# 9vvqaq/Indoor-Point-Cloud-Datasets-Controllable-Generation-Method-for-Mobile-Robots-3D-Scene-Perception

Measured on AMD Instinct MI355X. Metric: rays/sec (whole node), 32-line x 2048-azimuth sweep, higher is better.
Workload: dtype f32

## Files before the change

### indoor-point-cloud-datasets-controllable-generation-method-for-mobile-robots-3d-scene-perception_amd/csrc/lidarcast.hip

```cpp
#include <hip/hip_runtime.h>

#include <chrono>
#include <cmath>
#include <cstdio>
#include <cstring>
#include <mutex>
#include <new>
#include <string>
#include <vector>

#include "../../include/lidarcast.h"
#include "lrc_bvh.h"
#include "lrc_bvh_device.h"
#include "lrc_qnodes.h"
#include "lrc_device.h"

using namespace lrcdev;

namespace {

thread_local std::string g_err;

int fail(int code, const std::string& msg) {
    g_err = msg;
// ... 78 lines not shown
    float4* d_prim_plane = nullptr;
    std::mutex plane_mutex;
    float4* d_slot_sphere = nullptr;
    uint4* d_nodes_q = nullptr;
    float4* d_nodes_n = nullptr;
    uint4* d_nodes_q4 = nullptr;
    float4* d_nodes_n4 = nullptr;
    uint64_t num_nodes4 = 0;
    float qbase[3] = {0, 0, 0}, qW[3] = {1, 1, 1}, qinvW[3] = {1, 1, 1};
    const lrc_grid* cur_grid = nullptr;
    lrc_scene_info info{};
    lrc_scan_options opts{};
    uint64_t launches = 0, rays = 0;
};

namespace {

struct RebuildParams {
    const double* __restrict__ poses16;
    const double* __restrict__ dirs_soa;
    const uint32_t* __restrict__ prims;
    uint32_t pps;
    uint64_t stride;
    uint32_t seg_len, tps, ntiles, nseg;
    const float4* __restrict__ plane;
    uint32_t num_prims;
    const uint32_t* __restrict__ tile_off;
    const uint64_t* __restrict__ super_base;
    float4* __restrict__ out_xyzl;
    uint64_t* __restrict__ counts;
    uint32_t skip_slab;
};

struct TraceParams {
    const float4* nodes;
    const float4* tris;
    const uint32_t* slot_prim;
    const uint32_t* slot_label;
    const float* slot_box;
    const float4* prim_plane;
    uint32_t num_nodes;
    const uint4* nodes_q;
    const float4* nodes_n;
    const uint4* nodes_q4;
    const float4* nodes_n4;
    uint32_t stack_cap;
    uint32_t tile_chunk_log2;
    uint32_t force_redo;
    uint64_t* chain_word;
    uint64_t chain_seq;
    struct Pre {
        uint32_t blocks;
        uint32_t rows_only;
        uint32_t sharded, own_blocks;
        uint64_t tile_base;
        const uint64_t* super_base;
        RebuildParams rq;
        uint64_t seg_len, tps, ntiles, nseg;
        const uint32_t* tile_off;
        const uint32_t* super_total;
        lrc_compact_io io;
    } pre;
    float qbase[3], qW[3], qinvW[3];
    const float* rays6;
    const uint64_t* seg_offsets;
    const double* seg_centers3;
    uint32_t num_segments;
    const double* poses16;
    const double* dirs3;
    const double* angles2;
    const uint8_t* keep_mask;
    uint32_t* stats;
    uint64_t rays_per_pose;
    uint64_t total;
    int has_center;
    double cx, cy, cz;
    double max_range;
    double min_range;
    const float* range_noise;
    int incident_mode;
    lrc_hits out;
};

__device__ __forceinline__ uint32_t xcd_tile_chunked(uint32_t b, uint32_t nwg, uint32_t klog) {
    const uint32_t k = klog - 1u;
    const uint32_t full = (nwg >> (k + 3u)) << (k + 3u);
    if (b >= full) return b;
    const uint32_t x = b & 7u, j = b >> 3;
    return ((((j >> k) << 3) + x) << k) | (j & ((1u << k) - 1u));
}

__device__ __forceinline__ uint32_t xcd_tile(uint32_t b, uint32_t nwg) {
#ifdef LRC_NO_XCD_REMAP
    return b;
#endif
// ... 53 lines not shown
    }
#pragma unroll
    for (int k = 0; k < R; ++k) {
        if (!keep[k]) continue;
        typedef __attribute__((address_space(4))) const double cdouble;
        cdouble* M = (cdouble*)(q.poses16 + (size_t)seg[k] * 16);
        V3 o, d, h, pt;
        d.x = (float)dgemm_row(da[k], db[k], dc[k], M[0], M[1], M[2]);
        d.y = (float)dgemm_row(da[k], db[k], dc[k], M[4], M[5], M[6]);
        d.z = (float)dgemm_row(da[k], db[k], dc[k], M[8], M[9], M[10]);
        o.x = (float)M[3]; o.y = (float)M[7]; o.z = (float)M[11];
        const V3 v0{pa[k].x, pa[k].y, pa[k].z}, ng{pb[k].x, pb[k].y, pb[k].z};
        const float den = dot3(ng, d);
        const uint32_t sgn = __float_as_uint(den) & 0x80000000u;
        const float t = xorsign(dot3(ng, sub3(v0, o)), sgn) / __builtin_fabsf(den);
        hit_point(o, d, t, h, pt);
        typedef float v4f __attribute__((ext_vector_type(4)));
        const v4f row = {pt.x, pt.y, pt.z, pa[k].w};
        __builtin_nontemporal_store(row, (v4f*)(q.out_xyzl + dst[k]));
    }
}

__device__ __forceinline__ void rebuild_counts(const RebuildParams& q, uint32_t first, uint32_t step) {
    if (!q.counts) return;
    const uint32_t nsuper = (q.ntiles + 1023u) / 1024u;
    for (uint32_t sg = first; sg < q.nseg; sg += step) {
        const uint64_t g0 = (uint64_t)sg * q.tps, g1 = g0 + q.tps;
        const uint64_t o0 = g0 >= q.ntiles ? q.super_base[nsuper] : q.super_base[g0 >> 10] + q.tile_off[g0];
        const uint64_t o1 = g1 >= q.ntiles ? q.super_base[nsuper] : q.super_base[g1 >> 10] + q.tile_off[g1];
        q.counts[sg] = o1 - o0;
    }
}

template <bool FILTER_ALWAYS, bool BY_PRIM = false>
__device__ __forceinline__ void write_back(const TraceParams& p, uint64_t gid, uint32_t tid, V3 o, V3 d, double cx,
                                           double cy, double cz, float tbest, uint32_t best_slot) {
    constexpr int GEN = FILTER_ALWAYS ? 1 : 0;
    bool keep = best_slot != 0xFFFFFFFFu;
    float t_out = __builtin_inff();
    uint32_t prim = LRC_INVALID_PRIM;
    float nx = 0.f, ny = 0.f, nz = 0.f, px = 0.f, py = 0.f, pz = 0.f;
    uint32_t label = 0;
    double inc = 0.0;
    float inten = 0.f;
    if (keep && p.range_noise) {
        tbest = tbest + p.range_noise[gid];
        keep = tbest > 0.0f;
    }
    if (keep) {
        V3 hh, pp;
        hit_point(o, d, tbest, hh, pp);
        const float hx = hh.x, hy = hh.y, hz = hh.z;
        px = pp.x; py = pp.y; pz = pp.z;
        const double ex = (double)px - cx, ey = (double)py - cy, ez = (double)pz - cz;
        const double dist = __builtin_sqrt((ex * ex + ey * ey) + ez * ez);
        if (p.has_center || GEN != 0) keep = dist < p.max_range;
        if (p.min_range > 0.0) keep = keep & (dist >= p.min_range);
        if (keep) {
            t_out = tbest;
            if (BY_PRIM) {
                prim = best_slot;
                label = __float_as_uint(p.prim_plane[(size_t)best_slot * 2].w);
            } else {
                prim = p.slot_prim[best_slot];
                label = p.slot_label[best_slot];
            }
            if (p.out.normal3 || p.out.intensity || (p.out.incident_deg && p.incident_mode == 1)) {
                float4 c;
                if (BY_PRIM) { const float4 g = p.prim_plane[(size_t)best_slot * 2 + 1]; c = make_float4(0.f, g.x, g.y, g.z); }
                else c = p.tris[(size_t)best_slot * 3 + 2];
                const float len = __builtin_sqrtf(fma_(c.w, c.w, fma_(c.z, c.z, c.y * c.y)));
                nx = c.y / len; ny = c.z / len; nz = c.w / len;
            }
            if (p.out.incident_deg) {
                if (p.incident_mode == 1) {
                    const double cs = __builtin_fabs(((double)hx * (double)nx + (double)hy * (double)ny) +
                                                     (double)hz * (double)nz);
                    inc = acos(cs < 1.0 ? cs : 1.0) * kRadToDeg;
                } else {
                    inc = acos(__builtin_fabs(ez / dist)) * kRadToDeg;
                }
            }
            if (p.out.intensity)
                inten = __builtin_fabsf(fma_(hz, nz, fma_(hy, ny, hx * nx)));
            if (!p.out.normal3) { nx = ny = nz = 0.f; }
        } else {
            px = py = pz = 0.f;
        }
    }
    if (p.out.tile_count) {
        const unsigned long long m = __ballot(keep);
        if ((tid & 63u) == 0) p.out.tile_count[gid >> 6] = (uint32_t)__popcll(m);
    }
    if (p.out.t) p.out.t[gid] = t_out;
    if (p.out.t_label) ((uint2*)p.out.t_label)[gid] = make_uint2(__float_as_uint(t_out), label);
    if (p.out.prim) p.out.prim[gid] = prim;
    if (p.out.normal3) { float* q = p.out.normal3 + gid * 3; q[0] = nx; q[1] = ny; q[2] = nz; }
    if (p.out.point3) { float* q = p.out.point3 + gid * 3; q[0] = px; q[1] = py; q[2] = pz; }
    if (p.out.sem) p.out.sem[gid] = (uint16_t)(label & 0xFFFFu);
    if (p.out.ins) p.out.ins[gid] = (uint16_t)(label >> 16);
    if (p.out.incident_deg) p.out.incident_deg[gid] = inc;
    if (p.out.intensity) p.out.intensity[gid] = inten;

}

constexpr int kStatsWords = 5;

__device__ __forceinline__ uint64_t super_prefix_wave(const uint32_t* __restrict__ total, uint64_t s, uint32_t lane) {
    uint64_t acc = 0;
    for (uint64_t j = lane; j < s; j += 64) acc += total[j];
#pragma unroll
    for (int d = 32; d >= 1; d >>= 1) acc += __shfl_xor(acc, d, 64);
    return acc;
}
__device__ __forceinline__ uint64_t super_prefix_thread(const uint32_t* __restrict__ total, uint64_t s) {
    uint64_t acc = 0;
    for (uint64_t j = 0; j < s; ++j) acc += total[j];
    return acc;
}

__device__ __forceinline__ void segment_count(const lrc_compact_io& io, uint64_t tps, uint64_t ntiles, uint64_t nseg, uint64_t sg,
// ... 53 lines not shown
#pragma unroll
    for (int r = 0; r < R; ++r) {
        const uint64_t tile = tile0 + r;
        const bool valid = tile < ntiles;
        t[r] = valid ? io.t[tile * 64 + lane] : __builtin_inff();
        off[r] = valid ? (uint64_t)tile_off[tile_base + tile] : 0u;
        if (super_base && valid) off[r] += super_base[(tile_base + tile) >> 10];
    }
    const uint64_t sbase = super_base ? 0ull : super_prefix_wave(super_total, tile0 >> 10, lane);
    float px[R], py[R], pz[R];
    uint32_t lab[R];
    unsigned long long m[R];
#pragma unroll
    for (int r = 0; r < R; ++r) {
        const bool keep = t[r] < __builtin_inff();
        m[r] = __ballot(keep);
        px[r] = py[r] = pz[r] = 0.0f;
        lab[r] = 0u;
        if (keep) {
            const uint64_t src = (tile0 + r) * 64 + lane;
            const float* sp = io.point3 + src * 3;
            px[r] = sp[0]; py[r] = sp[1]; pz[r] = sp[2];
            lab[r] = (io.sem ? (uint32_t)io.sem[src] : 0u) | ((io.ins ? (uint32_t)io.ins[src] : 0u) << 16);
        }
    }
#pragma unroll
    for (int r = 0; r < R; ++r) {
        if (t[r] < __builtin_inff()) {
            const uint64_t dst = sbase + off[r] + (uint64_t)__popcll(m[r] & ((1ull << lane) - 1ull));
            ((float4*)io.out_xyzl)[dst] = make_float4(px[r], py[r], pz[r], __uint_as_float(lab[r]));
        }
    }
}
#ifndef LRC_PRE_TILES
#define LRC_PRE_TILES 8
#endif
constexpr int kPreTiles = LRC_PRE_TILES;

template <int I> struct IntTag { static constexpr int value = I; };

template <int GEN, int LEAFW, bool UNI, bool SPEC, bool STATS = false, int QN = 0>
__global__ __launch_bounds__(kTBlock, (QN != 0 && !STATS && GEN == 1) ? 8 : 1) void trace_kernel(const TraceParams p) {
    extern __shared__ int s_stack[];
    const uint32_t tid = threadIdx.x;
    if (GEN == 1 && p.pre.blocks != 0u && p.pre.sharded != 0u) {
        if (blockIdx.x < p.pre.blocks) {
            rebuild_counts(p.pre.rq, blockIdx.x * kTBlock + tid, p.pre.blocks * kTBlock);
            if (blockIdx.x < p.pre.own_blocks) {
                const uint64_t tile0 = (uint64_t)blockIdx.x * kPreTiles;
                if (tile0 < p.pre.ntiles)
                    scatter_tiles_xyzl<kPreTiles>(p.pre.io, p.pre.ntiles, tile0, tid, p.pre.tile_off, nullptr, p.pre.tile_base,
                                                  p.pre.super_base);
            } else {
                const uint32_t tile0 = (blockIdx.x - p.pre.own_blocks) * (uint32_t)LRC_REBUILD_R;
                if (tile0 < p.pre.rq.ntiles) rebuild_tiles<LRC_REBUILD_R>(p.pre.rq, tile0, p.pre.rq.ntiles, tid);
            }
            return;
        }
    } else
    if (GEN == 1 && p.pre.blocks != 0u) {
        if (blockIdx.x < p.pre.blocks) {
            if (p.pre.io.counts) segment_count(p.pre.io, p.pre.tps, p.pre.ntiles, p.pre.nseg, (uint64_t)blockIdx.x * kTBlock + tid,
                                               p.pre.tile_off, nullptr, p.pre.super_total);
            const uint64_t tile0 = (uint64_t)blockIdx.x * kPreTiles;
            if (tile0 < p.pre.ntiles) {
                if (p.pre.rows_only) {
                    scatter_tiles_xyzl<kPreTiles>(p.pre.io, p.pre.ntiles, tile0, tid, p.pre.tile_off, p.pre.super_total);
                } else {
                    for (int r = 0; r < kPreTiles; ++r)
                        if (tile0 + r < p.pre.ntiles)
                            scatter_tile(p.pre.io, p.pre.seg_len, p.pre.tps, tile0 + r, tid, p.pre.tile_off, nullptr, 0, p.pre.super_total);
                }
            }
            return;
        }
    }
    const uint32_t tile = p.tile_chunk_log2 ? xcd_tile_chunked(blockIdx.x - p.pre.blocks, gridDim.x - p.pre.blocks, p.tile_chunk_log2)
                                            : xcd_tile(blockIdx.x - p.pre.blocks, gridDim.x - p.pre.blocks);
    const uint64_t gid = (uint64_t)tile * kTBlock + tid;
    if (p.chain_word != nullptr && blockIdx.x == gridDim.x - 1 && tid == 0)
        __hip_atomic_store(p.chain_word, p.chain_seq, __ATOMIC_RELAXED, __HIP_MEMORY_SCOPE_SYSTEM);
    if (gid >= p.total) return;

    V3 o, d;
    double cx, cy, cz;
    bool live = true;
    uint32_t pose32 = 0;
    if (GEN == 1) {
        const uint64_t pose = gid / p.rays_per_pose;
        const uint64_t i = gid - pose * p.rays_per_pose;
        gen_ray(p.poses16, p.dirs3, pose, i, o, d, cx, cy, cz);
        pose32 = (uint32_t)pose;
    } else if (GEN == 2) {
        const uint64_t pose = gid / p.rays_per_pose;
        const double2 a = ((const double2*)p.angles2)[gid];
        gen_ray_angles(p.poses16, pose, a.x, a.y, o, d, cx, cy, cz);
        if (p.keep_mask) live = p.keep_mask[gid] != 0;
        pose32 = (uint32_t)pose;
    } else {
        const float* r = p.rays6 + gid * 6;
        o.x = r[0]; o.y = r[1]; o.z = r[2];
        d.x = r[3]; d.y = r[4]; d.z = r[5];
        if (p.keep_mask) live = p.keep_mask[gid] != 0;
        if (!p.seg_offsets && p.seg_centers3) {
// ... 505 lines not shown
}

__global__ __launch_bounds__(64) void compact_base_kernel(const uint32_t* super_total, uint64_t* super_base,
                                                          uint64_t nsuper) {
    const uint32_t lane = threadIdx.x;
    uint64_t carry = 0;
    for (uint64_t base = 0; base < nsuper; base += 64) {
        const uint64_t i = base + lane;
        const uint64_t v = i < nsuper ? super_total[i] : 0;
        uint64_t incl = v;
#pragma unroll
        for (int d = 1; d < 64; d <<= 1) {
            const uint64_t up = __shfl_up(incl, d, 64);
            if (lane >= (uint32_t)d) incl += up;
        }
        if (i < nsuper) super_base[i] = carry + incl - v;
        carry += __shfl(incl, 63, 64);
    }
    if (lane == 0) super_base[nsuper] = carry;
}

__global__ __launch_bounds__(kBlock) void compact_scatter_kernel(const lrc_compact_io io,
                                                                 uint64_t seg_len, uint64_t tps,
                                                                 uint64_t ntiles, uint64_t nseg,
                                                                 const uint32_t* tile_off,
                                                                 const uint64_t* super_base, uint64_t tile_base,
                                                                 const uint32_t* super_total) {
    if (io.counts) segment_count(io, tps, ntiles, nseg, (uint64_t)blockIdx.x * kBlock + threadIdx.x, tile_off, super_base, super_total);
    const uint64_t tile = (uint64_t)blockIdx.x * (kBlock / 64) + (threadIdx.x >> 6);
    if (tile >= ntiles) return;
    scatter_tile(io, seg_len, tps, tile, threadIdx.x & 63u, tile_off, super_base, tile_base, super_total);
}

__global__ __launch_bounds__(kBlock) void rows_range_kernel(const float4* __restrict__ rows, uint64_t n, float* __restrict__ out) {
    const uint64_t i = (uint64_t)blockIdx.x * kBlock + threadIdx.x;
    if (i >= n) return;
    const float4 r = rows[i];
    out[i] = __builtin_sqrtf((r.x * r.x + r.y * r.y) + r.z * r.z);
}


__global__ __launch_bounds__(kBlock) void cloud_count_kernel(const uint2* tl, uint64_t seg_len, uint64_t tps,
                                                             uint64_t ntiles, uint32_t* tile_cnt) {
    const uint64_t tile = (uint64_t)blockIdx.x * (kBlock / 64) + (threadIdx.x >> 6);
    if (tile >= ntiles) return;
    const uint64_t seg = tile / tps, chunk = tile - seg * tps;
    const uint64_t i = chunk * 64 + (threadIdx.x & 63u);
    bool keep = false;
    if (i < seg_len) keep = __uint_as_float(tl[seg * seg_len + i].x) < __builtin_inff();
    const unsigned long long m = __ballot(keep);
    if ((threadIdx.x & 63u) == 0) tile_cnt[tile] = (uint32_t)__popcll(m);
}

__global__ __launch_bounds__(kBlock) void cloud_scatter_kernel(const double* poses16, const double* dirs3,
                                                               const uint2* tl, uint64_t seg_len, uint64_t tps,
                                                               uint64_t ntiles, uint64_t nseg,
                                                               const uint32_t* tile_off, const uint64_t* super_base,
                                                               float4* out_xyzl, uint64_t* counts) {
    const uint32_t lane = threadIdx.x & 63u;
    if (counts) {
        const uint64_t sg = (uint64_t)blockIdx.x * kBlock + threadIdx.x;
        if (sg < nseg) {
            const uint64_t nsuper = (ntiles + 1023) / 1024;
            const uint64_t g0 = sg * tps, g1 = g0 + tps;
            const uint64_t o0 = g0 >= ntiles ? super_base[nsuper] : super_base[g0 >> 10] + tile_off[g0];
            const uint64_t o1 = g1 >= ntiles ? super_base[nsuper] : super_base[g1 >> 10] + tile_off[g1];
// ... 978 lines not shown
        ctx->compact_used[set] = true;
    }
    lrc_ctx::TileScratch& sc = ctx->compact_scratch[set];
    if (sc.tile_cap < ntiles + 1 && sc.d_tile_off) {
        LRC_HIP(hipEventSynchronize(ctx->compact_done[set]));
    }
    *out_set = set;
    return ensure_tile_scratch(ctx, sc, ntiles);
}

static int ensure_tile_scratch(lrc_ctx* ctx, lrc_ctx::TileScratch& sc, uint64_t ntiles) {
    (void)ctx;
    if (sc.tile_cap >= ntiles + 1) return LRC_OK;
    if (sc.d_tile_off) { (void)hipFree(sc.d_tile_off); sc.d_tile_off = nullptr; }
    if (sc.d_tile_cnt) { (void)hipFree(sc.d_tile_cnt); sc.d_tile_cnt = nullptr; }
    if (sc.d_super_total) { (void)hipFree(sc.d_super_total); sc.d_super_total = nullptr; }
    if (sc.d_super_base) { (void)hipFree(sc.d_super_base); sc.d_super_base = nullptr; }
    sc.tile_cap = 0;
    LRC_HIP(hipMalloc((void**)&sc.d_tile_off, (ntiles + 1) * 4));
    LRC_HIP(hipMalloc((void**)&sc.d_tile_cnt, (ntiles + 1) * 4));
    LRC_HIP(hipMalloc((void**)&sc.d_super_total, ((ntiles + 1023) / 1024 + 1) * 4));
    LRC_HIP(hipMalloc((void**)&sc.d_super_base, ((ntiles + 1023) / 1024 + 1) * 8));
    sc.tile_cap = ntiles + 1;
    return LRC_OK;
}

struct lrc_pipe {
    lrc_scene* scene = nullptr;
    int device = 0;
    uint64_t max_poses = 0, rays_per_pose = 0, cap = 0;
    static constexpr int kSets = 4;
    void* slab[kSets] = {};
    lrc_hits rec[kSets] = {};
    lrc_compact_io out[kSets] = {};
    uint64_t poses[kSets] = {};
    bool pending[kSets] = {};
    lrc_ctx::TileScratch scratch[2];
    hipStream_t s_trace[2] = {};
    hipEvent_t ev_in[kSets] = {}, ev_t0[kSets] = {}, ev_trace[kSets] = {}, ev_flush[2] = {};
    bool fused = true;
    uint64_t ticket = 0;
    lrc_ctx::TileScratch gscratch[2];
    double* d_dirs_soa = nullptr;
    const double* soa_of = nullptr;
};

int lrc_pipe_destroy(lrc_pipe* pp) {
    if (!pp) return LRC_OK;
    (void)hipSetDevice(pp->device);
    for (hipStream_t st : {pp->s_trace[0], pp->s_trace[1]})
        if (st) { (void)hipStreamSynchronize(st); (void)hipStreamDestroy(st); }
    for (int k = 0; k < lrc_pipe::kSets; ++k) {
        if (pp->slab[k]) (void)hipFree(pp->slab[k]);
        for (hipEvent_t e : {pp->ev_in[k], pp->ev_t0[k], pp->ev_trace[k]}) if (e) (void)hipEventDestroy(e);
    }
    for (int k = 0; k < 2; ++k) {
        if (pp->ev_flush[k]) (void)hipEventDestroy(pp->ev_flush[k]);
        for (lrc_ctx::TileScratch* scp : {&pp->scratch[k], &pp->gscratch[k]}) {
            lrc_ctx::TileScratch& sc = *scp;
            if (sc.d_tile_off) (void)hipFree(sc.d_tile_off);
            if (sc.d_tile_cnt) (void)hipFree(sc.d_tile_cnt);
            if (sc.d_super_total) (void)hipFree(sc.d_super_total);
            if (sc.d_super_base) (void)hipFree(sc.d_super_base);
        }
    }
    if (pp->d_dirs_soa) (void)hipFree(pp->d_dirs_soa);
    delete pp;
    return LRC_OK;
}

int lrc_pipe_create(lrc_scene* s, uint64_t max_poses, uint64_t rays_per_pose, lrc_pipe** out_pipe) {
    if (!out_pipe) return fail(LRC_ERR_INVALID_ARG, "lrc_pipe_create: out_pipe is NULL");
    *out_pipe = nullptr;
    if (!s) return fail(LRC_ERR_INVALID_ARG, "lrc_pipe_create: scene is NULL");
    if (max_poses == 0 || rays_per_pose == 0) return fail(LRC_ERR_INVALID_ARG, "lrc_pipe_create: max_poses and rays_per_pose must be positive");
    if (max_poses > 0x7FFFFFFFull || max_poses * rays_per_pose / rays_per_pose != max_poses || max_poses * rays_per_pose > (1ull << 36))
        return fail(LRC_ERR_INVALID_ARG, "lrc_pipe_create: batch too large");
    LRC_HIP(hipSetDevice(s->ctx->device));
    lrc_pipe* pp = new (std::nothrow) lrc_pipe();
    if (!pp) return fail(LRC_ERR_OOM, "lrc_pipe_create: out of host memory");
    pp->scene = s;
    pp->device = s->ctx->device;
    pp->max_poses = max_poses;
    pp->rays_per_pose = rays_per_pose;
    const uint64_t n = pp->cap = max_poses * rays_per_pose;
    const uint64_t tiles = max_poses * ((rays_per_pose + 63) / 64);
    pp->fused = rays_per_pose % 64 == 0 && (tiles + 1023) / 1024 <= 512;
    auto bail = [&](int rc) { (void)lrc_pipe_destroy(pp); return rc; };
    auto up = [](uint64_t b) { return (b + 255) & ~255ull; };
    const uint64_t off_t = 0, off_prim = off_t + up(4 * n), off_nrm = off_prim + up(4 * n), off_pt = off_nrm + up(12 * n),
                   off_sem = off_pt + up(12 * n), off_ins = off_sem + up(2 * n), off_tc = off_ins + up(2 * n),
                   bytes = off_tc + up(4 * ((n + 63) / 64));
    for (int k = 0; k < lrc_pipe::kSets; ++k) {
        hipError_t e = hipMalloc(&pp->slab[k], bytes);
        if (e != hipSuccess) { (void)hipGetLastError(); return bail(fail(LRC_ERR_OOM, "lrc_pipe_create: out of device memory for the record sets")); }
        char* b = (char*)pp->slab[k];
        lrc_hits& h = pp->rec[k];
        h.t = (float*)(b + off_t); h.prim = (uint32_t*)(b + off_prim); h.normal3 = (float*)(b + off_nrm);
        h.point3 = (float*)(b + off_pt); h.sem = (uint16_t*)(b + off_sem); h.ins = (uint16_t*)(b + off_ins);
        h.tile_count = (uint32_t*)(b + off_tc);
    }
    int prio_least = 0, prio_greatest = 0;
    if (hipDeviceGetStreamPriorityRange(&prio_least, &prio_greatest) != hipSuccess) return bail(fail(LRC_ERR_HIP, "lrc_pipe_create: stream priorities"));
    for (int k = 0; k < 2; ++k) {
        if (hipStreamCreateWithPriority(&pp->s_trace[k], hipStreamNonBlocking, prio_least) != hipSuccess) return bail(fail(LRC_ERR_HIP, "lrc_pipe_create: stream"));
        if (hipEventCreateWithFlags(&pp->ev_flush[k], hipEventDisableTiming) != hipSuccess) return bail(fail(LRC_ERR_HIP, "lrc_pipe_create: event"));
        int rc = ensure_tile_scratch(s->ctx, pp->scratch[k], tiles);
        if (rc) return bail(rc);
    }
    for (int k = 0; k < lrc_pipe::kSets; ++k) {
        if (hipEventCreateWithFlags(&pp->ev_in[k], hipEventDisableTiming) != hipSuccess ||
            hipEventCreate(&pp->ev_t0[k]) != hipSuccess || hipEventCreate(&pp->ev_trace[k]) != hipSuccess)
            return bail(fail(LRC_ERR_HIP, "lrc_pipe_create: event"));
    }
    *out_pipe = pp;
    return LRC_OK;
}

namespace {
lrc_compact_io pipe_io(const lrc_pipe* pp, int set) {
    lrc_compact_io io = pp->out[set];
    const lrc_hits& h = pp->rec[set];
    io.t = h.t; io.point3 = h.point3; io.sem = h.sem; io.ins = h.ins; io.incident_deg = nullptr; io.tile_count = h.tile_count;
    return io;
}
}

int lrc_pipe_submit(lrc_pipe* pp, const double* d_poses16, uint64_t P, const double* d_dirs3, double max_range,
                    const lrc_compact_io* d_out, void* stream, uint64_t* out_ticket) {
    if (!pp || !d_out) return fail(LRC_ERR_INVALID_ARG, "lrc_pipe_submit: NULL pipe or output");
    if (P == 0) { if (out_ticket) *out_ticket = pp->ticket; return LRC_OK; }
    if (P > pp->max_poses) return fail(LRC_ERR_INVALID_ARG, "lrc_pipe_submit: more poses than the pipeline was created for");
    if (!d_poses16 || !d_dirs3) return fail(LRC_ERR_INVALID_ARG, "lrc_pipe_submit: poses16 or dirs3 is NULL");
    if (d_out->out_incident_deg) return fail(LRC_ERR_INVALID_ARG, "lrc_pipe_submit: the pipeline's records carry no incident angle");
    lrc_scene* s = pp->scene;
    LRC_HIP(hipSetDevice(s->ctx->device));
    const uint64_t k = pp->ticket;
    const int set = (int)(k % lrc_pipe::kSets), lane = (int)(k % 2);
    hipStream_t T = pp->s_trace[lane];
    LRC_HIP(hipEventRecord(pp->ev_in[set], (hipStream_t)stream));
    LRC_HIP(hipStreamWaitEvent(T, pp->ev_in[set], 0));
    const uint64_t N = pp->rays_per_pose;
    TraceParams p{};
    p.poses16 = d_poses16;
    p.dirs3 = d_dirs3;
    p.rays_per_pose = N;
    p.total = P * N;
    p.has_center = 1;
    p.max_range = max_range;
    p.out = pp->rec[set];
    const int prev = (int)((k + lrc_pipe::kSets - 2) % lrc_pipe::kSets);
    lrc_compact_io pio{};
    if (pp->fused && k >= 2 && pp->pending[prev]) {
        pio = pipe_io(pp, prev);
        const uint64_t tps = N / 64, ntiles = pp->poses[prev] * tps;
        const uint64_t need = pio.counts ? (pp->poses[prev] + kTBlock - 1) / kTBlock : 0;
        const uint64_t tile_blocks = (ntiles + kPreTiles - 1) / kPreTiles;
        p.pre.blocks = (uint32_t)(tile_blocks > need ? tile_blocks : need);
        p.pre.rows_only = (pio.out_xyzl && !pio.out_point3 && !pio.out_sem && !pio.out_ins && !pio.out_index && !pio.out_range_origin) ? 1u : 0u;
        p.pre.seg_len = N; p.pre.tps = tps; p.pre.ntiles = ntiles; p.pre.nseg = pp->poses[prev];
        p.pre.tile_off = pp->scratch[lane].d_tile_off;
        p.pre.super_total = pp->scratch[lane].d_super_total;
        p.pre.io = pio;
    }
    LRC_HIP(hipEventRecord(pp->ev_t0[set], T));
    int rc = launch_trace(s, p, 1, T);
    if (rc) return rc;
    LRC_HIP(hipEventRecord(pp->ev_trace[set], T));
    if (p.pre.blocks) pp->pending[prev] = false;
    pp->out[set] = *d_out;
    pp->poses[set] = P;
    if (pp->fused) {
        const uint64_t ntiles = P * (N / 64), nsuper = (ntiles + 1023) / 1024;
#ifndef LRC_PIPE_SCAN_WAVES
#define LRC_PIPE_SCAN_WAVES 64
#endif
        hipLaunchKernelGGL(compact_scan_kernel, dim3((uint32_t)(nsuper < LRC_PIPE_SCAN_WAVES ? nsuper : LRC_PIPE_SCAN_WAVES)), dim3(64), 0, T, (const uint32_t*)pp->rec[set].tile_count,
                           ntiles, (uint64_t)0, pp->scratch[lane].d_tile_off, ntiles, pp->scratch[lane].d_super_total);
        LRC_HIP(hipGetLastError());
        pp->pending[set] = true;
    } else {
        lrc_compact_io io = pipe_io(pp, set);
        rc = enqueue_compaction(pp->scratch[lane], P, N, &io, T);
        if (rc) return rc;
    }
    pp->ticket = k + 1;
    if (out_ticket) *out_ticket = k + 1;
    return LRC_OK;
}

namespace {
int check_gathered(const lrc_pipe* pp, const lrc_gathered* g, const char* who) {
    auto bad = [&](const char* m) { return fail(LRC_ERR_INVALID_ARG, std::string(who) + ": " + m); };
    if (!g->d_all_poses16 || !g->d_all_prims || !g->d_all_tile_counts || !g->d_out_xyzl) return bad("NULL member of lrc_gathered");
    if (g->poses_per_slab == 0 || g->poses_per_slab > pp->max_poses || g->num_poses_all == 0 || g->num_poses_all % g->poses_per_slab)
        return bad("num_poses_all must be a multiple of poses_per_slab (<= the pipeline's max_poses)");
    if (g->own_slab >= g->num_poses_all / g->poses_per_slab) return bad("own_slab outside the gathered slabs");
    if (g->slab_stride_bytes % 4 || g->slab_stride_bytes < g->poses_per_slab * pp->rays_per_pose * 4) return bad("slab stride smaller than a slab");
    if (g->own_ticket == 0 || g->own_ticket > pp->ticket || pp->ticket - g->own_ticket >= (uint64_t)lrc_pipe::kSets)
        return bad("the own records of that scan are gone (four sets rotate): assemble within three submits");
    const uint64_t ntiles = g->num_poses_all * (pp->rays_per_pose / 64);
    if (ntiles > 0x7FFFFFFFull) return bad("too many entries");
    return LRC_OK;
}

int scan_gathered(lrc_pipe* pp, const lrc_gathered* g, const double* d_dirs3, hipStream_t st, int scan_waves) {
    lrc_scene* s = pp->scene;
    lrc_ctx::TileScratch& sc = pp->gscratch[g->scan_slot & 1u];
    const uint64_t N = pp->rays_per_pose, tps = N / 64, ntiles = g->num_poses_all * tps;
    int rc = ensure_tile_scratch(s->ctx, sc, ntiles);
    if (rc) return rc;
    if ((rc = ensure_prim_plane(s, st))) return rc;
    if (pp->soa_of != d_dirs3) {
        if (!pp->d_dirs_soa) LRC_HIP(hipMalloc((void**)&pp->d_dirs_soa, N * 24));
        hipLaunchKernelGGL(dirs_transpose_kernel, dim3((uint32_t)((N + kBlock - 1) / kBlock)), dim3(kBlock), 0, st, d_dirs3, (uint32_t)N,
                           pp->d_dirs_soa);
        LRC_HIP(hipStreamSynchronize(st));
        pp->soa_of = d_dirs3;
    }
    const uint64_t stride = g->slab_stride_bytes / 4, nsuper = (ntiles + 1023) / 1024;
    const uint64_t grid = scan_waves > 0 && nsuper > (uint64_t)scan_waves ? (uint64_t)scan_waves : nsuper;
    hipLaunchKernelGGL(compact_scan_kernel, dim3((uint32_t)grid), dim3(64), 0, st, g->d_all_tile_counts, g->poses_per_slab * tps, stride,
                       sc.d_tile_off, ntiles, sc.d_super_total);
    hipLaunchKernelGGL(compact_base_kernel, dim3(1), dim3(64), 0, st, (const uint32_t*)sc.d_super_total, sc.d_super_base, nsuper);
    LRC_HIP(hipGetLastError());
    return LRC_OK;
}

int prepare_gathered(lrc_pipe* pp, const lrc_gathered* g, RebuildParams* q, lrc_compact_io* own_io, uint64_t* own_tiles,
                     uint64_t* tile_base) {
    lrc_scene* s = pp->scene;
    lrc_ctx::TileScratch& sc = pp->gscratch[g->scan_slot & 1u];
    const uint64_t N = pp->rays_per_pose, tps = N / 64, ntiles = g->num_poses_all * tps;
// ... 34 lines not shown
    hipStream_t T = pp->s_trace[lane];
    LRC_HIP(hipEventRecord(pp->ev_in[set], (hipStream_t)stream));
    LRC_HIP(hipStreamWaitEvent(T, pp->ev_in[set], 0));
    const uint64_t N = pp->rays_per_pose;
    TraceParams p{};
    p.poses16 = d_poses16; p.dirs3 = d_dirs3; p.rays_per_pose = N; p.total = P * N; p.has_center = 1; p.max_range = max_range;
    p.out = pp->rec[set];
    p.out.prim = d_send_prim;
    p.out.tile_count = d_send_tile_count;
    lrc_compact_io own_io{};
    if (assemble) {
        uint64_t own_tiles = 0, tile_base = 0;
        if ((rc = prepare_gathered(pp, assemble, &p.pre.rq, &own_io, &own_tiles, &tile_base))) return rc;
        p.pre.sharded = 1;
        p.pre.io = own_io;
        p.pre.ntiles = own_tiles;
        p.pre.seg_len = N; p.pre.tps = N / 64;
        p.pre.tile_off = pp->gscratch[assemble->scan_slot & 1u].d_tile_off;
        p.pre.super_base = pp->gscratch[assemble->scan_slot & 1u].d_super_base;
        p.pre.tile_base = tile_base;
        p.pre.own_blocks = (uint32_t)((own_tiles + kPreTiles - 1) / kPreTiles);
        const uint64_t rb = ((uint64_t)p.pre.rq.ntiles + LRC_REBUILD_R - 1) / LRC_REBUILD_R;
        const uint64_t need = ((uint64_t)p.pre.rq.nseg + kTBlock - 1) / kTBlock;
        uint64_t blocks = p.pre.own_blocks + rb;
        if (blocks < need) blocks = need;
        p.pre.blocks = (uint32_t)blocks;
    }
    LRC_HIP(hipEventRecord(pp->ev_t0[set], T));
    rc = launch_trace(s, p, 1, T);
    if (rc) return rc;
    LRC_HIP(hipEventRecord(pp->ev_trace[set], T));
    pp->out[set] = lrc_compact_io{};
    pp->poses[set] = P;
    pp->pending[set] = false;
    pp->ticket = k + 1;
    if (out_ticket) *out_ticket = k + 1;
    return LRC_OK;
}

int lrc_pipe_trace_done(lrc_pipe* pp, uint64_t ticket, void* stream) {
    if (!pp) return fail(LRC_ERR_INVALID_ARG, "lrc_pipe_trace_done: pipe is NULL");
    if (ticket == 0 || ticket > pp->ticket || pp->ticket - ticket >= (uint64_t)lrc_pipe::kSets)
        return fail(LRC_ERR_INVALID_ARG, "lrc_pipe_trace_done: the events of that submit have been reused");
    LRC_HIP(hipSetDevice(pp->scene->ctx->device));
    LRC_HIP(hipStreamWaitEvent((hipStream_t)stream, pp->ev_trace[(ticket - 1) % lrc_pipe::kSets], 0));
    return LRC_OK;
}

int lrc_pipe_scan_gathered(lrc_pipe* pp, const double* d_dirs3, const lrc_gathered* g, void* stream) {
    if (!pp || !g || !d_dirs3) return fail(LRC_ERR_INVALID_ARG, "lrc_pipe_scan_gathered: NULL argument");
    int rc = check_gathered(pp, g, "lrc_pipe_scan_gathered");
    if (rc) return rc;
    LRC_HIP(hipSetDevice(pp->device));
    return scan_gathered(pp, g, d_dirs3, (hipStream_t)stream, LRC_PIPE_SCAN_WAVES * 4);
}

int lrc_pipe_assemble(lrc_pipe* pp, const double* d_dirs3, const lrc_gathered* g, void* stream) {
    if (!pp || !g || !d_dirs3) return fail(LRC_ERR_INVALID_ARG, "lrc_pipe_assemble: NULL argument");
    int rc = check_gathered(pp, g, "lrc_pipe_assemble");
    if (rc) return rc;
    LRC_HIP(hipSetDevice(pp->scene->ctx->device));
    hipStream_t st = (hipStream_t)stream;
    LRC_HIP(hipStreamWaitEvent(st, pp->ev_trace[(g->own_ticket - 1) % lrc_pipe::kSets], 0));
    RebuildParams q{};
    lrc_compact_io io{};
    uint64_t own_tiles = 0, tile_base = 0;
    if ((rc = prepare_gathered(pp, g, &q, &io, &own_tiles, &tile_base))) return rc;
    constexpr int kR = LRC_REBUILD_R;
    const uint64_t wblocks = (((uint64_t)q.ntiles + kR - 1) / kR + kBlock / 64 - 1) / (kBlock / 64);
    hipLaunchKernelGGL(prim_scatter_kernel<kR>, dim3((uint32_t)(wblocks ? wblocks : 1)), dim3(kBlock), 0, st, q);
    const uint64_t N = pp->rays_per_pose, tps = N / 64;
    const uint64_t nblocks = (own_tiles + kBlock / 64 - 1) / (kBlock / 64);
    if (nblocks)
        hipLaunchKernelGGL(compact_scatter_kernel, dim3((uint32_t)nblocks), dim3(kBlock), 0, st, io, N, tps, own_tiles, own_tiles / tps,
                           (const uint32_t*)q.tile_off, (const uint64_t*)q.super_base, tile_base, (const uint32_t*)nullptr);
    LRC_HIP(hipGetLastError());
    return LRC_OK;
}

int lrc_pipe_wait(lrc_pipe* pp, void* stream) {
    if (!pp) return fail(LRC_ERR_INVALID_ARG, "lrc_pipe_wait: pipe is NULL");
    if (pp->ticket == 0) return LRC_OK;
    LRC_HIP(hipSetDevice(pp->scene->ctx->device));
    for (uint64_t back = 2; back >= 1; --back) {
        if (pp->ticket < back) continue;
        const uint64_t k = pp->ticket - back;
        const int set = (int)(k % lrc_pipe::kSets), lane = (int)(k % 2);
        if (!pp->pending[set]) continue;
        lrc_compact_io io = pipe_io(pp, set);
        const uint64_t N = pp->rays_per_pose, tps = N / 64, ntiles = pp->poses[set] * tps;
        const uint64_t nblocks = (ntiles + kBlock / 64 - 1) / (kBlock / 64);
        const uint64_t need = io.counts ? (pp->poses[set] + kBlock - 1) / kBlock : 0;
        hipLaunchKernelGGL(compact_scatter_kernel, dim3((uint32_t)(nblocks > need ? nblocks : need)), dim3(kBlock), 0, pp->s_trace[lane],
                           io, N, tps, ntiles, pp->poses[set], (const uint32_t*)pp->scratch[lane].d_tile_off,
                           (const uint64_t*)nullptr, (uint64_t)0, (const uint32_t*)pp->scratch[lane].d_super_total);
        LRC_HIP(hipGetLastError());
        pp->pending[set] = false;
    }
    for (int lane = 0; lane < 2; ++lane) {
        LRC_HIP(hipEventRecord(pp->ev_flush[lane], pp->s_trace[lane]));
        LRC_HIP(hipStreamWaitEvent((hipStream_t)stream, pp->ev_flush[lane], 0));
    }
    return LRC_OK;
}

int lrc_pipe_records(lrc_pipe* pp, uint64_t ticket, lrc_hits* out_records) {
    if (!pp || !out_records) return fail(LRC_ERR_INVALID_ARG, "lrc_pipe_records: NULL argument");
    if (ticket == 0 || ticket > pp->ticket || pp->ticket - ticket >= (uint64_t)lrc_pipe::kSets)
        return fail(LRC_ERR_INVALID_ARG, "lrc_pipe_records: the records of that submit are gone (four sets rotate)");
    *out_records = pp->rec[(ticket - 1) % lrc_pipe::kSets];
    return LRC_OK;
}

int lrc_pipe_trace_ms(lrc_pipe* pp, uint64_t ticket, float* out_ms) {
    if (!pp || !out_ms) return fail(LRC_ERR_INVALID_ARG, "lrc_pipe_trace_ms: NULL argument");
    if (ticket == 0 || ticket > pp->ticket || pp->ticket - ticket >= (uint64_t)lrc_pipe::kSets)
        return fail(LRC_ERR_INVALID_ARG, "lrc_pipe_trace_ms: the events of that submit have been reused");
    const int set = (int)((ticket - 1) % lrc_pipe::kSets);
    LRC_HIP(hipSetDevice(pp->scene->ctx->device));
    LRC_HIP(hipEventSynchronize(pp->ev_trace[set]));
    LRC_HIP(hipEventElapsedTime(out_ms, pp->ev_t0[set], pp->ev_trace[set]));
    return LRC_OK;
}

int lrc_cloud_from_ranges_dev(lrc_ctx* ctx, const double* d_poses16, uint64_t P, const double* d_dirs3,
                              uint64_t N, const void* d_t_label, float* d_out_xyzl, uint64_t* d_counts,
                              void* stream) {
    if (!ctx) return fail(LRC_ERR_INVALID_ARG, "lrc_cloud_from_ranges_dev: ctx is NULL");
    if (P == 0 || N == 0) return LRC_OK;
    if (!d_poses16 || !d_dirs3 || !d_t_label || !d_out_xyzl)
        return fail(LRC_ERR_INVALID_ARG, "lrc_cloud_from_ranges_dev: NULL argument");
    LRC_HIP(hipSetDevice(ctx->device));
    hipStream_t st = (hipStream_t)stream;
    const uint64_t tps = (N + 63) / 64, ntiles = P * tps;
    const uint64_t nblocks = (ntiles + kBlock / 64 - 1) / (kBlock / 64);
    if (nblocks > 0x7FFFFFFFull) return fail(LRC_ERR_INVALID_ARG, "lrc_cloud_from_ranges_dev: too many entries");
    lrc_ctx::TileScratch& sc = ctx->cloud_scratch;
    int rc = ensure_tile_scratch(ctx, sc, ntiles);
    if (rc) return rc;
    const uint64_t nsuper = (ntiles + 1023) / 1024;
    hipLaunchKernelGGL(cloud_count_kernel, dim3((uint32_t)nblocks), dim3(kBlock), 0, st, (const uint2*)d_t_label, N,
                       tps, ntiles, sc.d_tile_cnt);
    hipLaunchKernelGGL(compact_scan_kernel, dim3((uint32_t)nsuper), dim3(64), 0, st,
// ... 692 lines not shown
```

Before: 12.96 billion.

## Write lean packed per-ray rows in fused pipe trace, expand full records lazily

In the fused pipeline, the trace kernel now writes only a packed float4 row (point plus label), a uint2 aux word (t and slot), and a per-tile keep mask, instead of the full record set (t, prim, normals, point, sem, ins). The compaction scatter reads these packed rows and masks. Full records are rebuilt by a new expand kernel only when lrc_pipe_records is called. This cuts per-ray write and read traffic in the trace and scatter stages, at the cost of extra buffers and a synchronous expansion if records are requested.

```diff
diff --git a/indoor-point-cloud-datasets-controllable-generation-method-for-mobile-robots-3d-scene-perception_amd/csrc/lidarcast.hip b/indoor-point-cloud-datasets-controllable-generation-method-for-mobile-robots-3d-scene-perception_amd/csrc/lidarcast.hip
--- a/indoor-point-cloud-datasets-controllable-generation-method-for-mobile-robots-3d-scene-perception_amd/csrc/lidarcast.hip
+++ b/indoor-point-cloud-datasets-controllable-generation-method-for-mobile-robots-3d-scene-perception_amd/csrc/lidarcast.hip
@@ -134,6 +134,11 @@
     uint32_t skip_slab;
 };
 
+struct LeanIn {
+    const float4* row;
+    const uint64_t* keep_mask;
+};
+
 struct TraceParams {
     const float4* nodes;
     const float4* tris;
@@ -162,7 +167,13 @@
         const uint32_t* tile_off;
         const uint32_t* super_total;
         lrc_compact_io io;
+        LeanIn lean;
     } pre;
+    struct Lean {
+        float4* row;
+        uint2* aux;
+        uint64_t* keep_mask;
+    } lean;
     float qbase[3], qW[3], qinvW[3];
     const float* rays6;
     const uint64_t* seg_offsets;
@@ -282,10 +293,16 @@
     }
 }
 
+__device__ __forceinline__ void slot_normal(float4 c, float& nx, float& ny, float& nz) {
+    const float len = __builtin_sqrtf(fma_(c.w, c.w, fma_(c.z, c.z, c.y * c.y)));
+    nx = c.y / len; ny = c.z / len; nz = c.w / len;
+}
+
 template <bool FILTER_ALWAYS, bool BY_PRIM = false>
 __device__ __forceinline__ void write_back(const TraceParams& p, uint64_t gid, uint32_t tid, V3 o, V3 d, double cx,
                                            double cy, double cz, float tbest, uint32_t best_slot) {
     constexpr int GEN = FILTER_ALWAYS ? 1 : 0;
+    const bool lean = FILTER_ALWAYS && !BY_PRIM && p.lean.row != nullptr;
     bool keep = best_slot != 0xFFFFFFFFu;
     float t_out = __builtin_inff();
     uint32_t prim = LRC_INVALID_PRIM;
@@ -306,7 +323,10 @@
         const double dist = __builtin_sqrt((ex * ex + ey * ey) + ez * ez);
         if (p.has_center || GEN != 0) keep = dist < p.max_range;
         if (p.min_range > 0.0) keep = keep & (dist >= p.min_range);
-        if (keep) {
+        if (keep && lean) {
+            t_out = tbest;
+            label = p.slot_label[best_slot];
+        } else if (keep) {
             t_out = tbest;
             if (BY_PRIM) {
                 prim = best_slot;
@@ -319,8 +339,7 @@
                 float4 c;
                 if (BY_PRIM) { const float4 g = p.prim_plane[(size_t)best_slot * 2 + 1]; c = make_float4(0.f, g.x, g.y, g.z); }
                 else c = p.tris[(size_t)best_slot * 3 + 2];
-                const float len = __builtin_sqrtf(fma_(c.w, c.w, fma_(c.z, c.z, c.y * c.y)));
-                nx = c.y / len; ny = c.z / len; nz = c.w / len;
+                slot_normal(c, nx, ny, nz);
             }
             if (p.out.incident_deg) {
                 if (p.incident_mode == 1) {
@@ -337,6 +356,16 @@
         } else {
             px = py = pz = 0.f;
         }
+    }
+    if (lean) {
+        const unsigned long long m = __ballot(keep);
+        if ((tid & 63u) == 0) {
+            if (p.out.tile_count) p.out.tile_count[gid >> 6] = (uint32_t)__popcll(m);
+            p.lean.keep_mask[gid >> 6] = m;
+        }
+        p.lean.row[gid] = make_float4(px, py, pz, __uint_as_float(label));
+        p.lean.aux[gid] = make_uint2(__float_as_uint(t_out), keep ? best_slot : 0xFFFFFFFFu);
+        return;
     }
     if (p.out.tile_count) {
         const unsigned long long m = __ballot(keep);
@@ -456,6 +485,59 @@
         }
     }
 }
+__device__ __forceinline__ void scatter_tile_lean(const lrc_compact_io& io, const LeanIn& in, uint64_t seg_len, uint64_t tps,
+                                                  uint64_t tile, uint32_t lane, const uint32_t* tile_off,
+                                                  const uint32_t* super_total) {
+    typedef __attribute__((address_space(4))) const uint64_t cu64;
+    const unsigned long long m = ((cu64*)in.keep_mask)[tile];
+    if (m == 0ull) return;
+    const uint64_t sbase = super_prefix_wave(super_total, tile >> 10, lane);
+    if (!((m >> lane) & 1ull)) return;
+    const uint64_t seg = tile / tps, i = (tile - seg * tps) * 64 + lane;
+    const float4 r = in.row[seg * seg_len + i];
+    const uint64_t dst = sbase + tile_off[tile] + (uint64_t)__popcll(m & ((1ull << lane) - 1ull));
+    const uint32_t lab = __float_as_uint(r.w);
+    if (io.out_xyzl) ((float4*)io.out_xyzl)[dst] = r;
+    if (io.out_point3) {
+        float* q = io.out_point3 + dst * 3;
+        q[0] = r.x; q[1] = r.y; q[2] = r.z;
+    }
+    if (io.out_sem) io.out_sem[dst] = (uint16_t)(lab & 0xFFFFu);
+    if (io.out_ins) io.out_ins[dst] = (uint16_t)(lab >> 16);
+    if (io.out_index) io.out_index[dst] = (uint32_t)i;
+    if (io.out_range_origin) io.out_range_origin[dst] = __builtin_sqrtf((r.x * r.x + r.y * r.y) + r.z * r.z);
+}
+
+template <int R>
+__device__ __forceinline__ void scatter_tiles_xyzl_lean(const lrc_compact_io& io, const LeanIn& in, uint64_t ntiles, uint64_t tile0,
+                                                        uint32_t lane, const uint32_t* tile_off, const uint32_t* super_total) {
+    typedef __attribute__((address_space(4))) const uint64_t cu64;
+    typedef __attribute__((address_space(4))) const uint32_t cu32;
+    constexpr int H = R < 4 ? R : 4;
+    static_assert(R % H == 0, "R: a multiple of four, or below four");
+    const uint64_t sbase = super_prefix_wave(super_total, tile0 >> 10, lane);
+    const unsigned long long below = (1ull << lane) - 1ull;
+#pragma unroll
+    for (int h = 0; h < R; h += H) {
+        unsigned long long m[H];
+        uint32_t off[H];
+#pragma unroll
+        for (int r = 0; r < H; ++r) {
+            const uint64_t tile = tile0 + h + r;
+            const bool valid = tile < ntiles;
+            m[r] = valid ? ((cu64*)in.keep_mask)[tile] : 0ull;
+            off[r] = valid ? ((cu32*)tile_off)[tile] : 0u;
+        }
+        float4 row[H];
+#pragma unroll
+        for (int r = 0; r < H; ++r)
+            row[r] = m[r] != 0ull ? in.row[(tile0 + h + r) * 64 + lane] : make_float4(0.f, 0.f, 0.f, 0.f);
+#pragma unroll
+        for (int r = 0; r < H; ++r)
+            if ((m[r] >> lane) & 1ull)
+                ((float4*)io.out_xyzl)[sbase + off[r] + (uint64_t)__popcll(m[r] & below)] = row[r];
+    }
+}
 #ifndef LRC_PRE_TILES
 #define LRC_PRE_TILES 8
 #endif
@@ -489,11 +571,13 @@
             const uint64_t tile0 = (uint64_t)blockIdx.x * kPreTiles;
             if (tile0 < p.pre.ntiles) {
                 if (p.pre.rows_only) {
-                    scatter_tiles_xyzl<kPreTiles>(p.pre.io, p.pre.ntiles, tile0, tid, p.pre.tile_off, p.pre.super_total);
+                    scatter_tiles_xyzl_lean<kPreTiles>(p.pre.io, p.pre.lean, p.pre.ntiles, tile0, tid, p.pre.tile_off,
+                                                       p.pre.super_total);
                 } else {
                     for (int r = 0; r < kPreTiles; ++r)
                         if (tile0 + r < p.pre.ntiles)
-                            scatter_tile(p.pre.io, p.pre.seg_len, p.pre.tps, tile0 + r, tid, p.pre.tile_off, nullptr, 0, p.pre.super_total);
+                            scatter_tile_lean(p.pre.io, p.pre.lean, p.pre.seg_len, p.pre.tps, tile0 + r, tid, p.pre.tile_off,
+                                              p.pre.super_total);
                 }
             }
             return;
@@ -1065,6 +1149,39 @@
     scatter_tile(io, seg_len, tps, tile, threadIdx.x & 63u, tile_off, super_base, tile_base, super_total);
 }
 
+__global__ __launch_bounds__(kBlock) void compact_scatter_lean_kernel(const lrc_compact_io io, const LeanIn in,
+                                                                      uint64_t seg_len, uint64_t tps,
+                                                                      uint64_t ntiles, uint64_t nseg,
+                                                                      const uint32_t* tile_off,
+                                                                      const uint32_t* super_total) {
+    if (io.counts) segment_count(io, tps, ntiles, nseg, (uint64_t)blockIdx.x * kBlock + threadIdx.x, tile_off, nullptr, super_total);
+    const uint64_t tile = (uint64_t)blockIdx.x * (kBlock / 64) + __builtin_amdgcn_readfirstlane(threadIdx.x >> 6);
+    if (tile >= ntiles) return;
+    scatter_tile_lean(io, in, seg_len, tps, tile, threadIdx.x & 63u, tile_off, super_total);
+}
+
+__global__ __launch_bounds__(kBlock) void expand_lean_kernel(const float4* __restrict__ row, const uint2* __restrict__ aux,
+                                                             const uint32_t* __restrict__ slot_prim, const float4* __restrict__ tris,
+                                                             lrc_hits out, uint64_t n) {
+    const uint64_t i = (uint64_t)blockIdx.x * kBlock + threadIdx.x;
+    if (i >= n) return;
+    const float4 r = row[i];
+    const uint2 a = aux[i];
+    const uint32_t lab = __float_as_uint(r.w);
+    uint32_t prim = LRC_INVALID_PRIM;
+    float nx = 0.f, ny = 0.f, nz = 0.f;
+    if (a.y != 0xFFFFFFFFu) {
+        prim = slot_prim[a.y];
+        slot_normal(tris[(size_t)a.y * 3 + 2], nx, ny, nz);
+    }
+    out.t[i] = __uint_as_float(a.x);
+    out.prim[i] = prim;
+    out.normal3[i * 3] = nx; out.normal3[i * 3 + 1] = ny; out.normal3[i * 3 + 2] = nz;
+    out.point3[i * 3] = r.x; out.point3[i * 3 + 1] = r.y; out.point3[i * 3 + 2] = r.z;
+    out.sem[i] = (uint16_t)(lab & 0xFFFFu);
+    out.ins[i] = (uint16_t)(lab >> 16);
+}
+
 __global__ __launch_bounds__(kBlock) void rows_range_kernel(const float4* __restrict__ rows, uint64_t n, float* __restrict__ out) {
     const uint64_t i = (uint64_t)blockIdx.x * kBlock + threadIdx.x;
     if (i >= n) return;
@@ -2109,12 +2226,17 @@
     static constexpr int kSets = 4;
     void* slab[kSets] = {};
     lrc_hits rec[kSets] = {};
+    float4* row[kSets] = {};
+    uint2* aux[kSets] = {};
+    uint64_t* keep_mask[kSets] = {};
+    bool lean[kSets] = {};
+    bool expanded[kSets] = {};
     lrc_compact_io out[kSets] = {};
     uint64_t poses[kSets] = {};
     bool pending[kSets] = {};
     lrc_ctx::TileScratch scratch[2];
     hipStream_t s_trace[2] = {};
-    hipEvent_t ev_in[kSets] = {}, ev_t0[kSets] = {}, ev_trace[kSets] = {}, ev_flush[2] = {};
+    hipEvent_t ev_in[kSets] = {}, ev_t0[kSets] = {}, ev_trace[kSets] = {}, ev_flush[2] = {}, ev_expand = nullptr;
     bool fused = true;
     uint64_t ticket = 0;
     lrc_ctx::TileScratch gscratch[2];
@@ -2131,6 +2253,7 @@
         if (pp->slab[k]) (void)hipFree(pp->slab[k]);
         for (hipEvent_t e : {pp->ev_in[k], pp->ev_t0[k], pp->ev_trace[k]}) if (e) (void)hipEventDestroy(e);
     }
+    if (pp->ev_expand) (void)hipEventDestroy(pp->ev_expand);
     for (int k = 0; k < 2; ++k) {
         if (pp->ev_flush[k]) (void)hipEventDestroy(pp->ev_flush[k]);
         for (lrc_ctx::TileScratch* scp : {&pp->scratch[k], &pp->gscratch[k]}) {
@@ -2167,7 +2290,8 @@
     auto up = [](uint64_t b) { return (b + 255) & ~255ull; };
     const uint64_t off_t = 0, off_prim = off_t + up(4 * n), off_nrm = off_prim + up(4 * n), off_pt = off_nrm + up(12 * n),
                    off_sem = off_pt + up(12 * n), off_ins = off_sem + up(2 * n), off_tc = off_ins + up(2 * n),
-                   bytes = off_tc + up(4 * ((n + 63) / 64));
+                   off_row = off_tc + up(4 * ((n + 63) / 64)), off_aux = off_row + (pp->fused ? up(16 * n) : 0),
+                   off_km = off_aux + (pp->fused ? up(8 * n) : 0), bytes = off_km + (pp->fused ? up(8 * ((n + 63) / 64)) : 0);
     for (int k = 0; k < lrc_pipe::kSets; ++k) {
         hipError_t e = hipMalloc(&pp->slab[k], bytes);
         if (e != hipSuccess) { (void)hipGetLastError(); return bail(fail(LRC_ERR_OOM, "lrc_pipe_create: out of device memory for the record sets")); }
@@ -2176,6 +2300,9 @@
         h.t = (float*)(b + off_t); h.prim = (uint32_t*)(b + off_prim); h.normal3 = (float*)(b + off_nrm);
         h.point3 = (float*)(b + off_pt); h.sem = (uint16_t*)(b + off_sem); h.ins = (uint16_t*)(b + off_ins);
         h.tile_count = (uint32_t*)(b + off_tc);
+        if (pp->fused) {
+            pp->row[k] = (float4*)(b + off_row); pp->aux[k] = (uint2*)(b + off_aux); pp->keep_mask[k] = (uint64_t*)(b + off_km);
+        }
     }
     int prio_least = 0, prio_greatest = 0;
     if (hipDeviceGetStreamPriorityRange(&prio_least, &prio_greatest) != hipSuccess) return bail(fail(LRC_ERR_HIP, "lrc_pipe_create: stream priorities"));
@@ -2190,6 +2317,7 @@
             hipEventCreate(&pp->ev_t0[k]) != hipSuccess || hipEventCreate(&pp->ev_trace[k]) != hipSuccess)
             return bail(fail(LRC_ERR_HIP, "lrc_pipe_create: event"));
     }
+    if (hipEventCreateWithFlags(&pp->ev_expand, hipEventDisableTiming) != hipSuccess) return bail(fail(LRC_ERR_HIP, "lrc_pipe_create: event"));
     *out_pipe = pp;
     return LRC_OK;
 }
@@ -2200,6 +2328,10 @@
     const lrc_hits& h = pp->rec[set];
     io.t = h.t; io.point3 = h.point3; io.sem = h.sem; io.ins = h.ins; io.incident_deg = nullptr; io.tile_count = h.tile_count;
     return io;
+}
+LeanIn pipe_lean(const lrc_pipe* pp, int set) {
+    if (!pp->lean[set]) return LeanIn{nullptr, nullptr};
+    return LeanIn{pp->row[set], pp->keep_mask[set]};
 }
 }
 
@@ -2226,6 +2358,9 @@
     p.has_center = 1;
     p.max_range = max_range;
     p.out = pp->rec[set];
+    if (pp->fused) {
+        p.lean.row = pp->row[set]; p.lean.aux = pp->aux[set]; p.lean.keep_mask = pp->keep_mask[set];
+    }
     const int prev = (int)((k + lrc_pipe::kSets - 2) % lrc_pipe::kSets);
     lrc_compact_io pio{};
     if (pp->fused && k >= 2 && pp->pending[prev]) {
@@ -2239,6 +2374,7 @@
         p.pre.tile_off = pp->scratch[lane].d_tile_off;
         p.pre.super_total = pp->scratch[lane].d_super_total;
         p.pre.io = pio;
+        p.pre.lean = pipe_lean(pp, prev);
     }
     LRC_HIP(hipEventRecord(pp->ev_t0[set], T));
     int rc = launch_trace(s, p, 1, T);
@@ -2247,6 +2383,8 @@
     if (p.pre.blocks) pp->pending[prev] = false;
     pp->out[set] = *d_out;
     pp->poses[set] = P;
+    pp->lean[set] = p.lean.row != nullptr;
+    pp->expanded[set] = false;
     if (pp->fused) {
         const uint64_t ntiles = P * (N / 64), nsuper = (ntiles + 1023) / 1024;
 #ifndef LRC_PIPE_SCAN_WAVES
@@ -2276,6 +2414,7 @@
     if (g->slab_stride_bytes % 4 || g->slab_stride_bytes < g->poses_per_slab * pp->rays_per_pose * 4) return bad("slab stride smaller than a slab");
     if (g->own_ticket == 0 || g->own_ticket > pp->ticket || pp->ticket - g->own_ticket >= (uint64_t)lrc_pipe::kSets)
         return bad("the own records of that scan are gone (four sets rotate): assemble within three submits");
+    if (pp->lean[(g->own_ticket - 1) % lrc_pipe::kSets]) return bad("own_ticket is not a submit of lrc_pipe_submit_sharded");
     const uint64_t ntiles = g->num_poses_all * (pp->rays_per_pose / 64);
     if (ntiles > 0x7FFFFFFFull) return bad("too many entries");
     return LRC_OK;
@@ -2376,6 +2515,8 @@
     LRC_HIP(hipEventRecord(pp->ev_trace[set], T));
     pp->out[set] = lrc_compact_io{};
     pp->poses[set] = P;
+    pp->lean[set] = false;
+    pp->expanded[set] = false;
     pp->pending[set] = false;
     pp->ticket = k + 1;
     if (out_ticket) *out_ticket = k + 1;
@@ -2435,9 +2576,15 @@
         const uint64_t N = pp->rays_per_pose, tps = N / 64, ntiles = pp->poses[set] * tps;
         const uint64_t nblocks = (ntiles + kBlock / 64 - 1) / (kBlock / 64);
         const uint64_t need = io.counts ? (pp->poses[set] + kBlock - 1) / kBlock : 0;
-        hipLaunchKernelGGL(compact_scatter_kernel, dim3((uint32_t)(nblocks > need ? nblocks : need)), dim3(kBlock), 0, pp->s_trace[lane],
-                           io, N, tps, ntiles, pp->poses[set], (const uint32_t*)pp->scratch[lane].d_tile_off,
-                           (const uint64_t*)nullptr, (uint64_t)0, (const uint32_t*)pp->scratch[lane].d_super_total);
+        const dim3 grid((uint32_t)(nblocks > need ? nblocks : need));
+        if (pp->lean[set])
+            hipLaunchKernelGGL(compact_scatter_lean_kernel, grid, dim3(kBlock), 0, pp->s_trace[lane], io, pipe_lean(pp, set), N, tps,
+                               ntiles, pp->poses[set], (const uint32_t*)pp->scratch[lane].d_tile_off,
+                               (const uint32_t*)pp->scratch[lane].d_super_total);
+        else
+            hipLaunchKernelGGL(compact_scatter_kernel, grid, dim3(kBlock), 0, pp->s_trace[lane],
+                               io, N, tps, ntiles, pp->poses[set], (const uint32_t*)pp->scratch[lane].d_tile_off,
+                               (const uint64_t*)nullptr, (uint64_t)0, (const uint32_t*)pp->scratch[lane].d_super_total);
         LRC_HIP(hipGetLastError());
         pp->pending[set] = false;
     }
@@ -2452,7 +2599,21 @@
     if (!pp || !out_records) return fail(LRC_ERR_INVALID_ARG, "lrc_pipe_records: NULL argument");
     if (ticket == 0 || ticket > pp->ticket || pp->ticket - ticket >= (uint64_t)lrc_pipe::kSets)
         return fail(LRC_ERR_INVALID_ARG, "lrc_pipe_records: the records of that submit are gone (four sets rotate)");
-    *out_records = pp->rec[(ticket - 1) % lrc_pipe::kSets];
+    const int set = (int)((ticket - 1) % lrc_pipe::kSets);
+    if (pp->lean[set] && !pp->expanded[set]) {
+        lrc_scene* s = pp->scene;
+        LRC_HIP(hipSetDevice(s->ctx->device));
+        hipStream_t T = pp->s_trace[(ticket - 1) % 2];
+        const uint64_t n = pp->poses[set] * pp->rays_per_pose;
+        hipLaunchKernelGGL(expand_lean_kernel, dim3((uint32_t)((n + kBlock - 1) / kBlock)), dim3(kBlock), 0, T,
+                           (const float4*)pp->row[set], (const uint2*)pp->aux[set], (const uint32_t*)s->d_slot_prim,
+                           (const float4*)s->d_tris, pp->rec[set], n);
+        LRC_HIP(hipGetLastError());
+        LRC_HIP(hipEventRecord(pp->ev_expand, T));
+        LRC_HIP(hipEventSynchronize(pp->ev_expand));
+        pp->expanded[set] = true;
+    }
+    *out_records = pp->rec[set];
     return LRC_OK;
 }
 
```

Result: faster. 13.65 billion, median of 6 (+5.3%).
